# tayloraswift/swift-png

Hardware: NVIDIA H100
Metric: MPixels/s decode (inflate+unfilter) (higher is better)
Workload: dtype u8

## Files before the change

include/pngb200.h:

```cpp
#ifndef PNGB200_H
#define PNGB200_H

#include <stddef.h>
#include <stdint.h>

#ifdef __cplusplus
extern "C" {
#endif

#define PNGB200_VERSION 1

typedef enum pngb200_status {
    PNGB200_OK                                   = 0,
    PNGB200_NEED_MORE_INPUT                      = 1,
    PNGB200_ERR_STREAM_CHECKSUM                  = -1,
    PNGB200_ERR_BLOCK_TYPE                       = -2,
    PNGB200_ERR_BLOCK_COUNT_PARITY               = -3,
    PNGB200_ERR_RUNLITERAL_SYMBOL_COUNT          = -4,
    PNGB200_ERR_CODELENGTH_HUFFMAN_TABLE         = -5,
    PNGB200_ERR_CODELENGTH_SEQUENCE              = -6,
    PNGB200_ERR_HUFFMAN_TABLE                    = -7,
    PNGB200_ERR_STRING_REFERENCE                 = -8,
    PNGB200_ERR_INVALID_SYMBOL                   = -9,
    PNGB200_ERR_ZLIB_METHOD                      = -16,
// ... 46 lines not shown

typedef struct pngb200_ctx pngb200_ctx;

pngb200_ctx* pngb200_ctx_create(int device);
void         pngb200_ctx_destroy(pngb200_ctx* ctx);
int          pngb200_ctx_trim(pngb200_ctx* ctx);
const char*  pngb200_last_error(const pngb200_ctx* ctx);
void*        pngb200_ctx_stream(pngb200_ctx* ctx);
int          pngb200_ctx_device(const pngb200_ctx* ctx);
uint64_t     pngb200_ctx_launch_count(const pngb200_ctx* ctx);
void         pngb200_ctx_set_inflate_mode(pngb200_ctx* ctx, int mode);
int          pngb200_ctx_stage_ms(pngb200_ctx* ctx, float ms[3]);
int          pngb200_ctx_inflate_stats(pngb200_ctx* ctx, size_t count, uint64_t out[4]);
int          pngb200_ctx_inflate_counters(pngb200_ctx* ctx, size_t count, uint64_t out[24]);
int          pngb200_ctx_segment_stats(pngb200_ctx* ctx, uint64_t out[3]);
int          pngb200_ctx_last_inflate_engine(pngb200_ctx* ctx);
int          pngb200_ctx_filter_histogram(pngb200_ctx* ctx, uint64_t out[6]);


typedef struct pngb200_stream_desc {
    const uint8_t* src;
    size_t         src_len;
    uint8_t*       dst;
    size_t         dst_cap;
    int32_t        format;
    int32_t        status;
    uint32_t       err_a, err_b;
    uint32_t       checksum;
    uint32_t       blocks;
    uint64_t       produced;
// ... 164 lines not shown
```

swift-png_b200/__init__.py:

```python
from __future__ import annotations

import ctypes as C
import importlib.util
import os
from dataclasses import dataclass

from . import shard

_HERE = os.path.dirname(os.path.abspath(__file__))
LIB_PATH = os.environ.get("PNGB200_LIB") or os.path.join(_HERE, "libpngb200.so")
HEADER_PATH = os.path.join(_HERE, "..", "include", "pngb200.h")

OK = 0
NEED_MORE_INPUT = 1
ERR_STREAM_CHECKSUM = -1
ERR_BLOCK_TYPE = -2
ERR_BLOCK_COUNT_PARITY = -3
ERR_RUNLITERAL_SYMBOL_COUNT = -4
ERR_CODELENGTH_HUFFMAN_TABLE = -5
ERR_CODELENGTH_SEQUENCE = -6
ERR_HUFFMAN_TABLE = -7
ERR_STRING_REFERENCE = -8
ERR_INVALID_SYMBOL = -9
ERR_ZLIB_METHOD = -16
# ... 178 lines not shown
    L.pngb200_ctx_inflate_stats.argtypes = [C.c_void_p, C.c_size_t, C.POINTER(C.c_uint64)]
    L.pngb200_ctx_inflate_stats.restype = C.c_int
    L.pngb200_deflator_create.argtypes = [C.c_void_p, C.c_int, C.c_int, C.c_int, C.c_size_t]
    L.pngb200_deflator_create.restype = C.c_void_p
    L.pngb200_deflator_destroy.argtypes = [C.c_void_p]
    L.pngb200_deflator_destroy.restype = None
    L.pngb200_deflator_push.argtypes = [C.c_void_p, C.c_char_p, C.c_size_t, C.c_int]
    L.pngb200_deflator_push.restype = C.c_int
    for fn in (L.pngb200_deflator_pop, L.pngb200_deflator_pull):
        fn.argtypes = [C.c_void_p, C.POINTER(C.POINTER(C.c_uint8)), C.POINTER(C.c_size_t)]
        fn.restype = C.c_int
    L.pngb200_ctx_filter_histogram.argtypes = [C.c_void_p, C.POINTER(C.c_uint64)]
    L.pngb200_ctx_filter_histogram.restype = C.c_int
    L.pngb200_ctx_segment_stats.argtypes = [C.c_void_p, C.POINTER(C.c_uint64)]
    L.pngb200_ctx_segment_stats.restype = C.c_int
    if os.environ.get("PNGB200_LIB") is None or hasattr(L, "pngb200_ctx_last_inflate_engine"):
        L.pngb200_ctx_last_inflate_engine.argtypes = [C.c_void_p]
        L.pngb200_ctx_last_inflate_engine.restype = C.c_int
    L.pngb200_ctx_inflate_counters.argtypes = [C.c_void_p, C.c_size_t, C.POINTER(C.c_uint64)]
    L.pngb200_ctx_inflate_counters.restype = C.c_int
    L.pngb200_inflate_batch.argtypes = [C.c_void_p, C.POINTER(StreamDesc), C.c_size_t, C.c_int]
    L.pngb200_inflate_batch.restype = C.c_int
    for name in ("pngb200_decode_batch", "pngb200_decode_batch_enqueue", "pngb200_unfilter_batch"):
        getattr(L, name).argtypes = [C.c_void_p, C.POINTER(ImageDesc), C.c_size_t, C.c_int]
        getattr(L, name).restype = C.c_int
    L.pngb200_decode_batch_finish.argtypes = [C.c_void_p, C.POINTER(ImageDesc), C.c_size_t]
    L.pngb200_decode_batch_finish.restype = C.c_int
    L.pngb200_filter_batch.argtypes = [C.c_void_p, C.POINTER(FilterDesc), C.c_size_t, C.c_int]
    L.pngb200_filter_batch.restype = C.c_int
    L.pngb200_deflate_batch.argtypes = [C.c_void_p, C.POINTER(DeflateDesc), C.c_size_t, C.c_int]
# ... 86 lines not shown
                 "stored_blocks"]
        return dict(waves=out[0], walk_tokens=out[1], resolve_rounds=out[2], fallbacks=out[3], tokens=out[4],
                    matches=out[5], deferred_matches=out[6], blocks=out[7],
                    cycles={n: out[8 + i] for i, n in enumerate(names)})

    def filter_histogram(self):
        out = (C.c_uint64 * 6)()
        self.check(self._lib.pngb200_ctx_filter_histogram(self.handle, out))
        return list(out)

    def segment_stats(self):
        out = (C.c_uint64 * 3)()
        self.check(self._lib.pngb200_ctx_segment_stats(self.handle, out))
        return dict(streams=out[0], segments=out[1], fallbacks=out[2])

    def last_inflate_engine(self) -> str:
        if not hasattr(self._lib, "pngb200_ctx_last_inflate_engine"):
            return ""
        return {0: "inflate_parallel_kernel", 1: "inflate_wave_kernel", 2: "inflate_cells_kernel"}.get(
            self._lib.pngb200_ctx_last_inflate_engine(self.handle), "")

    def set_inflate_mode(self, mode: int):
        self._lib.pngb200_ctx_set_inflate_mode(self.handle, mode)

    def check(self, rc: int):
        if rc != OK:
            raise PNGB200Error(rc, self._lib.pngb200_last_error(self.handle).decode())


@dataclass
# ... 358 lines not shown
```

swift-png_b200/csrc/common.cuh:

```cuda
#pragma once

#ifdef PNGB200_EMU
#include "simt.h"
#else
#include <cuda_runtime.h>
#define PNGB200_DYN_SMEM(name) extern __shared__ __align__(16) unsigned char name[]
#endif
#include <stdint.h>

#include "../../include/pngb200.h"

namespace pngb200 {

struct StreamJob {
    const uint8_t* src;
    uint64_t       src_len;
    uint8_t*       dst;
    uint64_t       dst_cap;
    uint64_t       start_bit;
    uint64_t       start_out;
    int32_t        format;
    int32_t        phase;
    uint64_t       stop_bit;
    uint32_t       symbolic;
    uint32_t       pad_;
    uint8_t*       scratch;
    uint64_t       scratch_cap;
};

struct StreamResult {
    int32_t  status;
    uint32_t err_a, err_b;
    uint32_t checksum;
    uint32_t blocks;
    uint32_t declared;
    uint64_t produced;
    uint64_t consumed_bits;
    uint64_t resume_bit;
    uint64_t resume_out;
    uint32_t trailer_seen;
    uint32_t phase;
    uint32_t stat_waves, stat_sync_rounds, stat_resolve_rounds, stat_fallback;
    uint64_t stat_tokens, stat_matches, stat_deferred;
    uint32_t ck_done;
    uint32_t pad_;
    uint64_t stat_cycles[12];
};

struct ImageJob {
    const uint8_t*      filtered;
    uint8_t*            pixels;
    const StreamResult* inflated;
    uint64_t            filtered_len;
    uint32_t            width, height;
    uint32_t            pitch;
    uint8_t             volume, depth, interlaced, bpp;
};

__device__ __forceinline__ uint64_t usable_bytes(const StreamResult* r, uint64_t fallback)
{
    if (r == nullptr) return fallback;
// ... 26 lines not shown
```

swift-png_b200/csrc/inflate_segments.cuh:

```cuda
#pragma once

#include "common.cuh"
#include "inflate_wave.cuh"

namespace pngb200 {

constexpr uint32_t SEG_WINDOW = 32768;

struct SegmentRecord {
    const uint16_t* sym;
    uint8_t*        out;
    uint64_t        produced;
    uint32_t        stream;
    uint32_t        first;
};

__global__ void __launch_bounds__(256) window_propagate_kernel(const SegmentRecord* segs, const uint32_t* stream_first,
                                                               uint32_t nstreams, uint8_t* windows)
{
    if (blockIdx.x >= nstreams) return;
    const uint32_t lo = stream_first[blockIdx.x], hi = stream_first[blockIdx.x + 1];
    for (uint32_t k = lo; k + 1 < hi; ++k) {
        const SegmentRecord s  = segs[k];
        const uint8_t*      w  = windows + (size_t)k * SEG_WINDOW;
// ... 31 lines not shown
        const uint64_t i = base + j;
        if (i >= s.produced) break;
        const uint16_t x = s.sym[i];
        s.out[i] = (x & 0x8000u) ? (s.first ? 0 : w[x & 0x7fffu]) : (uint8_t)x;
    }
}

struct SplitRecord {
    const StreamResult* head;
    const StreamResult* tail;
    const uint16_t*     sym;
    uint8_t*            out;
    uint64_t            dst_cap;
    uint64_t            split_bit;
    StreamResult*       final_;
};

constexpr uint32_t SPLIT_CTAS = 64;

__device__ __forceinline__ bool split_lines_up(const SplitRecord& s, uint64_t n1, uint64_t n2)
{
    return s.head->status == PNGB200_OK && s.head->phase == 1 && s.head->consumed_bits == s.split_bit &&
           s.tail->status == PNGB200_OK && s.tail->phase == 2 && n1 >= SEG_WINDOW && n1 + n2 <= s.dst_cap;
}

__global__ void __launch_bounds__(256) split_resolve_kernel(const SplitRecord* recs, uint32_t* partial)
{
    const SplitRecord s  = recs[blockIdx.x];
    const uint64_t    n1 = s.head->produced, n2 = s.tail->produced;
    uint32_t*         pp = partial + 2 * ((size_t)blockIdx.x * SPLIT_CTAS + blockIdx.y);
    if (!split_lines_up(s, n1, n2)) return;
    const uint8_t* w = s.out + n1 - SEG_WINDOW;
    uint8_t*       o = s.out + n1;
    uint64_t a = 0, b = 0;
    for (uint64_t base = (uint64_t)blockIdx.y * 4096; base < n2; base += (uint64_t)SPLIT_CTAS * 4096) {
        for (uint32_t j = threadIdx.x; j < 4096; j += blockDim.x) {
            const uint64_t i = base + j;
            if (i >= n2) break;
            const uint16_t x = s.sym[i];
            const uint8_t  v = (x & 0x8000u) ? w[x & 0x7fffu] : (uint8_t)x;
            o[i] = v;
            a += v;
            b += (n2 - i) * v;
        }
        b %= ADLER_MOD32;
    }
    uint32_t a32 = (uint32_t)(a % ADLER_MOD32), b32 = (uint32_t)b;
    for (int k = 16; k; k >>= 1) {
        a32 += __shfl_down_sync(0xffffffffu, a32, k);
        b32 += __shfl_down_sync(0xffffffffu, b32, k);
    }
    __shared__ uint32_t red[2][8];
    const unsigned warp = threadIdx.x >> 5;
    if (lane_id() == 0) { red[0][warp] = a32 % ADLER_MOD32; red[1][warp] = b32 % ADLER_MOD32; }
    __syncthreads();
    if (threadIdx.x == 0) {
        uint32_t sa = 0, sb = 0;
        for (unsigned k = 0; k < blockDim.x / 32; ++k) { sa += red[0][k]; sb += red[1][k]; }
// ... 48 lines not shown
```

swift-png_b200/csrc/inflate_wave.cuh:

```cuda
#pragma once

#include "inflate_serial.cuh"

namespace pngb200 {

#ifndef WV_CTAS
#define WV_CTAS 2
#endif
constexpr int      WV_THREADS      = 256;
constexpr int      WV_CTAS_PER_SM  = WV_CTAS;
constexpr int      WV_WARPS        = WV_THREADS / 32;
constexpr uint32_t WV_SUB_BITS     = 256;
constexpr uint32_t WV_BITS         = WV_THREADS * WV_SUB_BITS;
constexpr uint32_t WV_WORDS        = WV_BITS / 32 + 8;
constexpr uint32_t WV_SMEM_WORDS   = WV_WORDS + WV_WORDS / 8 + 1;
constexpr uint32_t WV_RING         = 65536;
constexpr uint32_t WV_WINDOW       = 32768;
constexpr uint32_t WV_OUT_BYTES    = WV_RING - WV_WINDOW;
constexpr uint32_t WV_BITMAP_WORDS = WV_OUT_BYTES / 32;
constexpr uint32_t WV_LIST_CAP     = WV_BITS / 2 + 64;
constexpr uint64_t WV_MAX_WAVE_OUT = (uint64_t)WV_LIST_CAP * 258;
constexpr uint32_t WV_HDR_WORDS    = 192;
constexpr uint32_t ADLER_MOD32     = 65521;
#ifndef WV_POLL_NS
// ... 35 lines not shown
    uint32_t     wn_[WV_THREADS];
    uint64_t     cross_[WV_THREADS];
    uint16_t     wc_[WV_THREADS];
    uint16_t     next_[WV_THREADS];
    uint8_t      kind_[WV_THREADS];
    uint8_t      wlist[2][WV_THREADS];
    uint16_t     dpre_[WV_THREADS];
    uint16_t     cst_[WV_THREADS];
    uint32_t     dsum[WV_WARPS];
    uint32_t     wcount[3];
    uint32_t     bitmap[WV_BITMAP_WORDS];
    uint8_t      ring[WV_RING] __align__(16);
    uint64_t     warp_sums[WV_WARPS + 1];
    uint32_t     adler_a[WV_WARPS], adler_b[WV_WARPS];
    uint32_t     exc[WV_WARPS], valid[WV_WARPS];
    uint32_t     last, term, anomaly, ticket;
    uint64_t     cyc[12], tick;
    uint64_t     pf_bar;
    WvHeader     hdr;
};

struct WvParams {
    const StreamJob* jobs;
    StreamResult*    results;
    const uint32_t*  order;
    uint32_t*        ticket;
    uint8_t*         scratch;
    uint64_t         scratch_stride;
    uint64_t         bitmap_words;
    int              count;
};

struct CopyItem { uint32_t o; uint32_t run_dist; };

#ifdef PNGB200_EMU
typedef uintptr_t saddr_t;
inline uint32_t lds32(saddr_t addr) { return *(const uint32_t*)addr; }
inline uint32_t bfe32(uint32_t x, uint32_t pos, uint32_t len);
inline saddr_t smem_addr(const void* p) { return (uintptr_t)p; }
inline saddr_t opaque(saddr_t a) { return a; }
inline uint32_t bmsk(uint32_t pos, uint32_t width)
{
    pos &= 0xff; width &= 0xff;
    if (pos > 31 || width == 0) return 0;
    const uint32_t m = width >= 32 ? ~0u : (1u << width) - 1u;
// ... 482 lines not shown
        }
        __syncthreads();
        if (sh.ticket >= (uint32_t)P.count) return;
        const int       j   = P.order ? (int)P.order[sh.ticket] : (int)sh.ticket;
        const StreamJob job = P.jobs[j];
        StreamResult*   r   = P.results + j;

        BitReader br;
        br.init(job.src, job.src_len, job.start_bit);
        uint64_t out    = job.start_out;
        uint32_t blocks = 0, waves = 0, resolve_rounds = 0;
        uint64_t n_tokens = 0, n_matches = 0, n_deferred = 0, walk_tokens = 0;
        int      st     = PNGB200_OK;
        uint32_t phase  = (uint32_t)job.phase;
        uint64_t resume_bit = job.start_bit, resume_out = job.start_out;
        uint8_t* const dst = job.dst;
        const bool     sym = job.symbolic != 0;
        const uint32_t esz = sym ? 2u : 1u;
        const uint32_t mis = (uint32_t)((uintptr_t)dst & 15);
        bool fallback = false;
        bool ring_stale = job.start_out != 0;
        bool     pf_pending = false;
        uint64_t pf_first = 0;
        const bool adler_on = job.start_out == 0 && !sym;
        uint32_t   s1 = 1, s2 = 0;
        uint64_t   pend_len = 0;
        bool       pend = false;
        auto fold_adler = [&]() {
            if (pend && t == 0) {
                uint64_t A = 0, B = 0;
                for (int w = 0; w < WV_WARPS; ++w) { A += sh.adler_a[w]; B += sh.adler_b[w]; }
                s2 = (uint32_t)((s2 + (pend_len % ADLER_MOD32) * s1 + B) % ADLER_MOD32);
                s1 = (uint32_t)((s1 + A) % ADLER_MOD32);
            }
            pend = false;
// ... 6 lines not shown
            uint32_t a32 = (uint32_t)(a % ADLER_MOD32), b32 = (uint32_t)(bw % ADLER_MOD32);
            for (int o = 16; o; o >>= 1) {
                a32 += __shfl_down_sync(0xffffffffu, a32, o);
                b32 += __shfl_down_sync(0xffffffffu, b32, o);
            }
            if (lane == 0) { sh.adler_a[warp] = a32; sh.adler_b[warp] = b32; }
            pend = true;
            pend_len = n;
        };
        auto tick = [&](int i) {
            if (t == 0) {
                const uint64_t now = (uint64_t)clock64();
                sh.cyc[i] += now - sh.tick;
                sh.tick = now;
            }
        };

        if (phase == 0) {
            st = read_stream_header(br, job.format, r);
            if (st == PNGB200_OK) {
                resume_bit = br.at();
                phase = 1;
            }
        }
        if (st == PNGB200_OK && phase == 2) st = read_trailer(br, job.format, r);

        while (st == PNGB200_OK && phase == 1) {
            __syncthreads();
            fold_adler();
            {
// ... 18 lines not shown
            }
            __syncthreads();
            const WvHeader hdr = sh.hdr;
            st = hdr.status;
            if (st != PNGB200_OK) break;
            const int      type = hdr.type, final = hdr.final;
            const uint32_t stored = hdr.stored;
            br.seek(hdr.pos);
            if (type != 0) {
                st = build_block_tables(&sh.ser, r, hdr.nlit, hdr.ndist, (int)t, WV_THREADS);
                if (st != PNGB200_OK) break;
            }
            tick(0);
            if (type == 0) {
                if (!br.have(8 * (uint64_t)stored)) { st = PNGB200_NEED_MORE_INPUT; break; }
                if (out + stored > job.dst_cap) { st = fail(r, PNGB200_ERR_OUTPUT_CAPACITY); break; }
                const uint8_t* s = job.src + (br.at() >> 3);
                if (sym) for (uint32_t k = t; k < stored; k += WV_THREADS) reinterpret_cast<uint16_t*>(dst)[out + k] = s[k];
                else for (uint32_t k = t; k < stored; k += WV_THREADS) dst[out + k] = s[k];
                if (adler_on && stored) adler_hbm(s, stored);
                if (stored) ring_stale = true;
                out += stored;
                br.seek(br.pos + 8 * (uint64_t)stored);
                __syncthreads();
                fold_adler();
                tick(9);
            } else {
                bool block_done = false;
                while (!block_done) {
                    ++waves;
                    const uint64_t wstart = br.pos;
                    const uint64_t wbase  = (wstart >> 5) & ~(uint64_t)7;
                    __syncthreads();
                    bool staged = false;
                    if (pf_pending) {
                        while (!mbar_try_wait(&sh.pf_bar, pf_parity)) {}
                        pf_parity ^= 1;
                        pf_pending = false;
                        if (wbase >= pf_first && wbase - pf_first < 4) {
                            const uint32_t* lin = sh.mask + (uint32_t)(wbase - pf_first);
// ... 221 lines not shown
                        uint64_t ws = lane < WV_WARPS ? sh.warp_sums[lane] : 0, wi = ws;
                        for (int o = 1; o < 32; o <<= 1) {
                            uint64_t v = __shfl_up_sync(0xffffffffu, wi, o);
                            if ((int)lane >= o) wi += v;
                        }
                        if (lane < WV_WARPS) sh.warp_sums[lane] = wi - ws;
                        if (lane == WV_WARPS - 1) sh.warp_sums[WV_WARPS] = wi;
                    }
                    __syncthreads();
                    tick(5);
                    const uint64_t excl    = sh.warp_sums[warp] + incl - mine;
                    const uint32_t o_start = (uint32_t)(excl & 0xffffffffffull);
                    const uint32_t c_start = (uint32_t)(excl >> 40);
                    const uint64_t total64 = sh.warp_sums[WV_WARPS] & 0xffffffffffull;
                    const uint32_t np      = (uint32_t)(sh.warp_sums[WV_WARPS] >> 40);
                    if (sh.anomaly || out + total64 > job.dst_cap || total64 > P.bitmap_words * 32) {
                        fallback = true;
                        break;
                    }
                    const uint32_t  total  = (uint32_t)total64;
                    {
                        const uint64_t nbase = wbase + WV_BITS / 32;
                        const uint64_t first = nbase - ((((uintptr_t)br.words >> 2) + nbase) & 3);
                        if (first >= 1 && (first + WV_PF_WORDS + 1) * 32 <= br.total_bits) {
                            if (t == 0) {
                                fence_proxy_async();
                                mbar_expect_tx(&sh.pf_bar, sizeof(uint32_t) * WV_PF_WORDS);
                                bulk_g2s(sh.mask, br.words + first, sizeof(uint32_t) * WV_PF_WORDS, &sh.pf_bar);
                            }
                            pf_pending = true;
                            pf_first = first;
                        }
// ... 107 lines not shown
                            ++rounds;
                            if (!__any_sync(0xffffffffu, g < nd)) break;
                            if (!__any_sync(0xffffffffu, progressed)) __nanosleep(WV_POLL_NS);
                        }
                        resolve_rounds += rounds;
                        WV_COUNT(4, rounds);
                    }
                    __threadfence_block();
                    __syncthreads();
                    tick(7);
                    if (sh.anomaly) {
                        for (uint32_t k = t; k < (total + 31) / 32; k += WV_THREADS) U[k] = 0;
                        fallback = true;
                        break;
                    }
                    if (!in_hbm && total) {
                        const uint32_t shift = rbase & 15u;
                        uint8_t* const gbase = wdst - shift;
                        const uint32_t rb16  = rbase - shift;
                        const uint32_t end   = shift + total;
                        const uint32_t nq    = (end + 15) >> 4;
                        uint32_t a = 0, bw = 0;
                        for (uint32_t c = t; c < nq; c += WV_THREADS) {
                            const uint32_t lo = c << 4, hi = lo + 16;
                            if (lo >= shift && hi <= end) {
                                const uint4 x = *reinterpret_cast<const uint4*>(sh.ring + ((rb16 + lo) & 0xffffu));
                                reinterpret_cast<uint4*>(gbase)[c] = x;
                                adler_chunk16_u32(x, end - lo, a, bw);
                            } else {
                                for (uint32_t k = max(lo, shift); k < min(hi, end); ++k) {
// ... 12 lines not shown
                            }
                            if (lane == 0) { sh.adler_a[warp] = a32; sh.adler_b[warp] = b32; }
                            pend = true;
                            pend_len = total;
                        }
                    } else if (in_hbm && adler_on) {
                        adler_hbm(wdst, total);
                    }
                    tick(8);
                    out += total;
                    if (t == 0) n_matches += np;
                    n_tokens += emitted;
                    n_deferred += deferred;
                    br.seek((wbase << 5) + sh.wpos_[last]);
                    if (term == WK_EOB || term == WK_OWN_EOB) block_done = true;
                }
                if (fallback) break;
            }
            ++blocks;
            resume_bit = br.at();
            resume_out = out;
            if (job.stop_bit && !final && br.at() >= job.stop_bit) break;
            if (final) {
                phase = 2;
                st = read_trailer(br, job.format, r);
                break;
            }
        }
        if (pf_pending) {
            while (!mbar_try_wait(&sh.pf_bar, pf_parity)) {}
// ... 25 lines not shown
                for (int w = 0; w < WV_WARPS; ++w) {
                    tk += sh.warp_sums[w];
                    df += sh.adler_a[w];
                    wt += sh.adler_b[w];
                    rr = max(rr, sh.exc[w]);
                }
                r->stat_waves          = waves;
                r->stat_sync_rounds    = (uint32_t)min(wt, (uint64_t)0xffffffffu);
                r->stat_resolve_rounds = rr;
                r->stat_tokens         = tk;
                r->stat_matches        = n_matches;
                r->stat_deferred       = df;
                for (int k = 0; k < 12; ++k) r->stat_cycles[k] = sh.cyc[k];
            }
        }
        if (fallback && sym) {
            if (t == 0) {
                r->status = PNGB200_ERR_INTERNAL;
                r->produced = out;
                r->consumed_bits = br.at();
                r->blocks = blocks;
            }
        } else if (fallback) {
            __syncthreads();
            if (warp == 0) serial_inflate(sh.ser, job, r, resume_bit, resume_out, 1, blocks);
        } else if (t == 0) {
            if (r->status == 0) r->status = st;
            r->produced      = out;
            r->consumed_bits = br.at();
            r->blocks        = blocks;
            r->resume_bit    = resume_bit;
            r->resume_out    = resume_out;
            r->phase         = phase;
            if (adler_on && job.format != PNGB200_FORMAT_GZIP) {
                const uint32_t computed = s2 << 16 | s1;
                r->checksum = computed;
                r->ck_done  = 1;
                if (r->trailer_seen && job.format != PNGB200_FORMAT_IOS && r->status >= 0 && r->declared != computed) {
                    r->status = PNGB200_ERR_STREAM_CHECKSUM;
                    r->err_a  = r->declared;
                    r->err_b  = computed;
                }
            }
        }
        if (t == 0) r->stat_fallback = fallback ? 1u : 0u;
    }
}

#ifndef PNGB200_EMU
inline int configure_inflate_wave()
{
    return (int)cudaFuncSetAttribute(inflate_wave_kernel, cudaFuncAttributeMaxDynamicSharedMemorySize,
                                     (int)sizeof(WvShared));
}
#endif

inline uint64_t wv_bitmap_words(uint64_t max_dst_cap)
{
    uint64_t bytes = max_dst_cap < WV_MAX_WAVE_OUT ? max_dst_cap : WV_MAX_WAVE_OUT;
    return (bytes + 31) / 32 + 8;
// ... 9 lines not shown
```

swift-png_b200/csrc/pngb200_api.cu:

```cuda
#include <cuda_runtime.h>

#include <algorithm>
#include <cstdarg>
#include <cstdio>
#include <cstdlib>
#include <cstring>
#include <functional>
#include <string>
#include <thread>
#include <vector>

#include "checksum.cuh"
#include "common.cuh"
#include "deflate.cuh"
#include "filter.cuh"
#include "color.cuh"
#include "crc32.cuh"
#include "inflate_wave.cuh"
#include "inflate_parallel.cuh"
#include "inflate_cells.cuh"
#include "block_search.cuh"
#include "inflate_segments.cuh"
#include "inflate_serial.cuh"
#include "unfilter.cuh"
// ... 66 lines not shown
    cudaStream_t stream = nullptr;
    uint64_t     launches = 0;
    int          inflate_mode = 0;
    int          last_engine = -1;
    bool         cells_auto = false;
    bool         cells_segments = true;
    int          sm_count = 132;
    size_t       device_bytes = 0;
    std::string  error;
    bool         pending = false;
    int          pending_memspace = 0;
    DevBuf d_jobs, d_results, d_imgjobs, d_genjobs, d_misc, d_partial, d_filtered, d_in, d_out, d_order, d_scratch, d_dfscratch, d_dfjobs, d_dfres, d_enc,
           d_file, d_crc, d_seg, d_crctab, d_sgjobs, d_sgres, d_sgsym, d_sgsearch, d_sgrec, d_sgwin;
    PinBuf h_jobs, h_results, h_imgjobs, h_genjobs, h_misc, h_order, h_crc, h_seg, h_sgsearch, h_sgjobs, h_sgres, h_sgrec;
    uint64_t seg_streams = 0, seg_segments = 0, seg_fallbacks = 0;
    uint64_t scratch_stride = 0;
    size_t parallel_threshold = 8192;
    unsigned long long* d_hist = nullptr;
    size_t peer_streams = 0;
    bool   split = true;
    size_t plan_slots = 0;
    cudaEvent_t ev[4] = {nullptr, nullptr, nullptr, nullptr};
    std::vector<uint64_t> expected;
    std::vector<size_t>   out_offset;
    std::vector<size_t>   out_bytes;
    std::vector<pngb200_ctx*> lanes;
    std::function<int()> bulk_h2d;
};

namespace {
// ... 219 lines not shown
        StreamResult* hf = ctx->h_sgres.as<StreamResult>();
        for (size_t a = 0; a < accepted.size(); ++a) {
            hf[a] = finals[a];
            CU(cudaMemcpyAsync(d_results + accepted[a], hf + a, sizeof(StreamResult), cudaMemcpyHostToDevice, ctx->stream));
        }
        std::vector<uint32_t> rest;
        for (uint32_t i : par)
            if (std::find(accepted.begin(), accepted.end(), i) == accepted.end()) rest.push_back(i);
        par.swap(rest);
    }
    return PNGB200_OK;
}

size_t plan_slots(const pngb200_ctx* ctx) { return ctx->plan_slots ? ctx->plan_slots : (size_t)ctx->sm_count * WV_CTAS_PER_SM; }

constexpr double kSymbolicCost = 1.38;


double split_head_share(const pngb200_ctx* ctx, const StreamJob* h_jobs, const std::vector<uint32_t>& par)
{
    constexpr uint64_t kMinSplit = 1u << 20;
    const size_t slots = plan_slots(ctx), nb = par.size();
    if (!ctx->split || ctx->peer_streams || nb * 2 <= slots || nb >= slots) return 0;
    const double h = nb * kSymbolicCost / ((double)(slots - nb) + nb * kSymbolicCost);
    if (h < 0.55 || h > 0.95) return 0;
    for (uint32_t i : par) {
        const StreamJob& j = h_jobs[i];
        if (j.format != PNGB200_FORMAT_ZLIB || j.start_bit != 0 || j.phase != 0 || j.src_len < kMinSplit || j.dst_cap < kMinSplit ||
            !j.scratch || (uintptr_t)j.scratch % 16 || (double)j.scratch_cap < 2.5 * (1.0 - h) * (double)j.dst_cap + 4096)
            return 0;
    }
// ... 9 lines not shown
    for (size_t k = 0; k < nb; ++k) {
        const StreamJob& j = h_jobs[par[k]];
        sj[k] = SearchJob{j.src, j.src_len, (uint64_t)(h * (double)(8 * j.src_len)), 8 * j.src_len, ~0ull};
    }
    CU(cudaMemcpyAsync(ctx->d_sgsearch.p, sj, sizeof(SearchJob) * nb, cudaMemcpyHostToDevice, ctx->stream));
    block_search_kernel<<<dim3((unsigned)nb, BS_CTAS), 256, 0, ctx->stream>>>(ctx->d_sgsearch.as<SearchJob>(), (uint32_t)nb);
    ctx->launches++;
    CU(cudaMemcpyAsync(sj, ctx->d_sgsearch.p, sizeof(SearchJob) * nb, cudaMemcpyDeviceToHost, ctx->stream));
    CU(cudaStreamSynchronize(ctx->stream));
    std::vector<uint32_t> cut, rest;
    for (size_t k = 0; k < nb; ++k) (sj[k].found != ~0ull ? cut : rest).push_back(par[k]);
    const size_t n = cut.size();
    if (n == 0) return PNGB200_OK;
    CU(ctx->h_sgjobs.reserve(sizeof(StreamJob) * 2 * n));
    CU(ctx->d_sgjobs.reserve(sizeof(StreamJob) * 2 * n));
    CU(ctx->d_sgres.reserve(sizeof(StreamResult) * 2 * n));
    StreamJob* sg = ctx->h_sgjobs.as<StreamJob>();
    uint64_t max_cap = 0;
    for (size_t k = 0, s = 0; k < nb; ++k) {
        if (sj[k].found == ~0ull) continue;
        const StreamJob& j = h_jobs[par[k]];
        StreamJob& hd = sg[s];
        StreamJob& tl = sg[n + s];
        ++s;
        hd = j;
        hd.stop_bit = sj[k].found;
        tl = j;
        tl.start_bit = sj[k].found;
        tl.phase = 1;
        tl.symbolic = 1;
        tl.dst = j.scratch;
        tl.dst_cap = j.scratch_cap / 2 - 64;
        max_cap = std::max(max_cap, j.dst_cap);
    }
    CU(cudaMemcpyAsync(ctx->d_sgjobs.p, sg, sizeof(StreamJob) * 2 * n, cudaMemcpyHostToDevice, ctx->stream));
    CU(cudaMemsetAsync(ctx->d_sgres.p, 0, sizeof(StreamResult) * 2 * n, ctx->stream));
    {
        WvParams pp;
        pp.bitmap_words = wv_bitmap_words(max_cap);
        pp.scratch_stride = wv_scratch_stride(pp.bitmap_words);
        const unsigned grid = (unsigned)std::min<size_t>(2 * n, slots);
        const size_t need = (size_t)pp.scratch_stride * grid + 256;
        if (need > ctx->d_scratch.cap || pp.scratch_stride != ctx->scratch_stride) {
            CU(ctx->d_scratch.reserve(need));
            CU(cudaMemsetAsync(ctx->d_scratch.p, 0, ctx->d_scratch.cap, ctx->stream));
            ctx->scratch_stride = pp.scratch_stride;
        }
        pp.ticket = (uint32_t*)((char*)ctx->d_scratch.p + (size_t)pp.scratch_stride * grid);
        CU(cudaMemsetAsync(pp.ticket, 0, sizeof(uint32_t), ctx->stream));
        pp.jobs = ctx->d_sgjobs.as<StreamJob>();
        pp.results = ctx->d_sgres.as<StreamResult>();
        pp.order = nullptr;
        pp.scratch = ctx->d_scratch.as<uint8_t>();
        pp.count = (int)(2 * n);
        inflate_wave_kernel<<<grid, WV_THREADS, sizeof(WvShared), ctx->stream>>>(pp);
        ctx->launches++;
    }
    const size_t off_accept  = align_up(sizeof(SplitRecord) * n, 256);
    const size_t off_partial = align_up(off_accept + sizeof(uint32_t) * n, 256);
    const size_t table       = off_partial + sizeof(uint32_t) * 2 * SPLIT_CTAS * n;
    CU(ctx->h_sgrec.reserve(off_partial));
    CU(ctx->d_sgrec.reserve(table));
    SplitRecord* rec = ctx->h_sgrec.as<SplitRecord>();
    const StreamResult* d_sgres = ctx->d_sgres.as<StreamResult>();
    for (size_t s = 0; s < n; ++s) {
        const StreamJob& j = h_jobs[cut[s]];
        rec[s] = SplitRecord{d_sgres + s, d_sgres + n + s, (const uint16_t*)j.scratch, j.dst, j.dst_cap, sg[s].stop_bit,
                             ctx->d_results.as<StreamResult>() + cut[s]};
    }
    CU(cudaMemcpyAsync(ctx->d_sgrec.p, rec, sizeof(SplitRecord) * n, cudaMemcpyHostToDevice, ctx->stream));
    const SplitRecord* d_rec = ctx->d_sgrec.as<SplitRecord>();
    uint32_t* d_accept  = (uint32_t*)((char*)ctx->d_sgrec.p + off_accept);
    uint32_t* d_partial = (uint32_t*)((char*)ctx->d_sgrec.p + off_partial);
    split_resolve_kernel<<<dim3((unsigned)n, SPLIT_CTAS), 256, 0, ctx->stream>>>(d_rec, d_partial);
    split_finish_kernel<<<(unsigned)((n + 127) / 128), 128, 0, ctx->stream>>>(d_rec, (uint32_t)n, d_partial, d_accept);
    ctx->launches += 2;
    CU(cudaGetLastError());
    uint32_t* accept = (uint32_t*)((char*)ctx->h_sgrec.p + off_accept);
    CU(cudaMemcpyAsync(accept, d_accept, sizeof(uint32_t) * n, cudaMemcpyDeviceToHost, ctx->stream));
    CU(cudaStreamSynchronize(ctx->stream));
    ctx->seg_streams += n;
    ctx->seg_segments += 2 * n;
    for (size_t s = 0; s < n; ++s)
        if (!accept[s]) {
            ctx->seg_fallbacks++;
            rest.push_back(cut[s]);
        }
    std::vector<uint32_t> left;
    for (uint32_t i : par)
        if (std::find(rest.begin(), rest.end(), i) != rest.end()) left.push_back(i);
    par.swap(left);
    return PNGB200_OK;
}

int run_inflate(pngb200_ctx* ctx, const StreamJob* h_jobs, size_t count)
{
    ctx->last_engine = -1;
    StreamJob*    d_jobs    = ctx->d_jobs.as<StreamJob>();
    StreamResult* d_results = ctx->d_results.as<StreamResult>();
    ctx->seg_streams = ctx->seg_segments = ctx->seg_fallbacks = 0;
    CU(cudaMemsetAsync(d_results, 0, sizeof(StreamResult) * count, ctx->stream));
    auto before_first_launch = [&]() -> int {
        int rc = PNGB200_OK;
        if (ctx->bulk_h2d) {
            rc = ctx->bulk_h2d();
            ctx->bulk_h2d = nullptr;
        }
        if (rc == PNGB200_OK) CU(cudaEventRecord(ctx->ev[0], ctx->stream));
        return rc;
    };
    {
        std::vector<uint32_t> par, ser;
        for (size_t i = 0; i < count; ++i) {
            bool big = h_jobs[i].src_len >= ctx->parallel_threshold;
            if (ctx->inflate_mode == 1) big = false;
// ... 530 lines not shown
    DeviceGuard guard(ctx->device);
    std::vector<pngb200_ctx*> all{ctx};
    all.insert(all.end(), ctx->lanes.begin(), ctx->lanes.end());
    for (pngb200_ctx* c : all) {
        if (!c->d_hist) continue;
        unsigned long long h[6];
        CU(cudaStreamSynchronize(c->stream));
        CU(cudaMemcpy(h, c->d_hist, sizeof h, cudaMemcpyDeviceToHost));
        for (int k = 0; k < 6; ++k) out[k] += h[k];
    }
    return PNGB200_OK;
}

int pngb200_ctx_last_inflate_engine(pngb200_ctx* ctx) { return ctx ? ctx->last_engine : -1; }

int pngb200_ctx_segment_stats(pngb200_ctx* ctx, uint64_t out[3])
{
    if (!ctx || !out) return PNGB200_ERR_BAD_ARGUMENT;
    out[0] = ctx->seg_streams;
    out[1] = ctx->seg_segments;
    out[2] = ctx->seg_fallbacks;
    return PNGB200_OK;
}

int pngb200_ctx_stage_ms(pngb200_ctx* ctx, float ms[3])
{
    if (!ctx || !ms) return PNGB200_ERR_BAD_ARGUMENT;
    DeviceGuard guard(ctx->device);
    for (int i = 0; i < 3; ++i)
        if (cudaEventElapsedTime(&ms[i], ctx->ev[i], ctx->ev[i + 1]) != cudaSuccess) {
// ... 32 lines not shown
                CU(cudaMemcpyAsync(ctx->d_in.as<uint8_t>() + in_off[i], s[i].src, s[i].src_len,
                                   cudaMemcpyHostToDevice, ctx->stream));
    }
    for (size_t i = 0; i < count; ++i) {
        bool host = memspace == PNGB200_MEM_HOST;
        jobs[i].src = host ? ctx->d_in.as<uint8_t>() + in_off[i] : s[i].src;
        jobs[i].src_len = s[i].src_len;
        jobs[i].dst = host ? ctx->d_out.as<uint8_t>() + out_off[i] : s[i].dst;
        jobs[i].dst_cap = s[i].dst_cap;
        jobs[i].start_bit = 0;
        jobs[i].start_out = 0;
        jobs[i].format = s[i].format;
        jobs[i].phase = 0;
        jobs[i].stop_bit = 0;
        jobs[i].symbolic = 0;
        jobs[i].pad_ = 0;
        jobs[i].scratch = nullptr;
        jobs[i].scratch_cap = 0;
    }
    CU(cudaMemcpyAsync(ctx->d_jobs.p, jobs, sizeof(StreamJob) * count, cudaMemcpyHostToDevice, ctx->stream));
    int rc = run_inflate(ctx, jobs, count);
    if (rc != PNGB200_OK) return rc;
    CU(cudaMemcpyAsync(ctx->h_results.p, ctx->d_results.p, sizeof(StreamResult) * count,
                       cudaMemcpyDeviceToHost, ctx->stream));
    CU(cudaStreamSynchronize(ctx->stream));
    const StreamResult* r = ctx->h_results.as<StreamResult>();
    for (size_t i = 0; i < count; ++i) {
        s[i].status = r[i].status;
        s[i].err_a = r[i].err_a;
        s[i].err_b = r[i].err_b;
        s[i].checksum = r[i].checksum;
// ... 53 lines not shown
            return PNGB200_OK;
        };
    }
    StreamJob* jobs = ctx->h_jobs.as<StreamJob>();
    for (size_t i = 0; i < count; ++i) {
        jobs[i].src = host ? ctx->d_in.as<uint8_t>() + in_off[i] : im[i].idat;
        jobs[i].src_len = im[i].idat_len;
        jobs[i].dst = ctx->d_filtered.as<uint8_t>() + f_off[i];
        jobs[i].dst_cap = geo[i].filtered + 16;
        jobs[i].start_bit = 0;
        jobs[i].start_out = 0;
        jobs[i].format = im[i].format;
        jobs[i].phase = 0;
        jobs[i].stop_bit = 0;
        jobs[i].symbolic = 0;
        jobs[i].pad_ = 0;
        jobs[i].scratch = host ? nullptr : im[i].pixels;
        jobs[i].scratch_cap = host ? 0 : im[i].pixels_cap;
    }
    CU(cudaMemcpyAsync(ctx->d_jobs.p, jobs, sizeof(StreamJob) * count, cudaMemcpyHostToDevice, ctx->stream));
    int rc = run_inflate(ctx, jobs, count);
    ctx->bulk_h2d = nullptr;
    if (rc != PNGB200_OK) return rc;
    std::vector<UnfilterItem> items(count);
    for (size_t i = 0; i < count; ++i) {
        UnfilterItem& it = items[i];
        it.filtered = jobs[i].dst;
        it.filtered_mut = jobs[i].dst;
        it.pixels = host ? ctx->d_out.as<uint8_t>() + ctx->out_offset[i] : im[i].pixels;
        it.inflated = ctx->d_results.as<StreamResult>() + i;
        it.filtered_len = 0;
// ... 599 lines not shown
    CU(z->h_res.reserve(sizeof(StreamResult) + sizeof(StreamJob)));
    int rc = inflator_grow_out(z, std::max<size_t>(1 << 16, z->produced + 4 * n + 1024));
    if (rc != PNGB200_OK) return rc;
    for (;;) {
        StreamJob* job = (StreamJob*)((char*)z->h_res.p + sizeof(StreamResult));
        job->src = z->d_in.as<uint8_t>();
        job->src_len = z->input.size();
        job->dst = z->d_out.as<uint8_t>();
        job->dst_cap = z->d_out.cap;
        job->start_bit = z->resume_bit;
        job->start_out = z->resume_out;
        job->format = z->format;
        job->phase = (int32_t)z->phase;
        job->stop_bit = 0;
        job->symbolic = 0;
        job->pad_ = 0;
        CU(cudaMemcpyAsync(z->d_job.p, job, sizeof(StreamJob), cudaMemcpyHostToDevice, ctx->stream));
        CU(cudaMemsetAsync(z->d_res.p, 0, sizeof(StreamResult), ctx->stream));
        const uint64_t pending = z->input.size() - std::min<uint64_t>(z->input.size(), z->resume_bit >> 3);
        if (pending >= (64u << 10)) {
            const uint64_t bitmap_words = wv_bitmap_words(job->dst_cap);
            const uint64_t stride = wv_scratch_stride(bitmap_words);
            const size_t   need = (size_t)stride + 256;
            if (need > ctx->d_scratch.cap || stride != ctx->scratch_stride) {
                CU(ctx->d_scratch.reserve(need));
                CU(cudaMemsetAsync(ctx->d_scratch.p, 0, ctx->d_scratch.cap, ctx->stream));
                ctx->scratch_stride = stride;
            }
            uint32_t* ticket = (uint32_t*)((char*)ctx->d_scratch.p + (size_t)stride);
            CU(cudaMemsetAsync(ticket, 0, sizeof(uint32_t), ctx->stream));
            WvParams pp;
// ... 95 lines not shown
```

Measured before the change: 9955.

## Let speculative tail inflate switch from symbolic to plain bytes once window resolved

The tail segment of a split stream is decoded symbolically (16-bit entries referencing the unknown head window). Once no unresolved back-references remain within the last window, the wave kernel now converts the last window to bytes and continues emitting plain 8-bit output into a fresh region of the scratch buffer, recording the switch point. The split resolve kernel then resolves only the symbolic prefix and copies the byte suffix with vectorized funnel-shift loads while folding Adler-32. This halves output traffic for the late part of the tail, at the cost of an extra per-wave max-mark reduction and a barrier. The symbolic cost constant used to size the head/tail split is lowered to match, and split statistics plus a host copy of the piece results are added.

```diff
diff --git a/include/pngb200.h b/include/pngb200.h
--- a/include/pngb200.h
+++ b/include/pngb200.h
@@ -84,6 +84,7 @@
 int          pngb200_ctx_inflate_stats(pngb200_ctx* ctx, size_t count, uint64_t out[4]);
 int          pngb200_ctx_inflate_counters(pngb200_ctx* ctx, size_t count, uint64_t out[24]);
 int          pngb200_ctx_segment_stats(pngb200_ctx* ctx, uint64_t out[3]);
+int          pngb200_ctx_split_stats(pngb200_ctx* ctx, uint64_t out[6]);
 int          pngb200_ctx_last_inflate_engine(pngb200_ctx* ctx);
 int          pngb200_ctx_filter_histogram(pngb200_ctx* ctx, uint64_t out[6]);
 
diff --git a/swift-png_b200/__init__.py b/swift-png_b200/__init__.py
--- a/swift-png_b200/__init__.py
+++ b/swift-png_b200/__init__.py
@@ -216,6 +216,9 @@
     L.pngb200_ctx_filter_histogram.restype = C.c_int
     L.pngb200_ctx_segment_stats.argtypes = [C.c_void_p, C.POINTER(C.c_uint64)]
     L.pngb200_ctx_segment_stats.restype = C.c_int
+    if os.environ.get("PNGB200_LIB") is None or hasattr(L, "pngb200_ctx_split_stats"):
+        L.pngb200_ctx_split_stats.argtypes = [C.c_void_p, C.POINTER(C.c_uint64)]
+        L.pngb200_ctx_split_stats.restype = C.c_int
     if os.environ.get("PNGB200_LIB") is None or hasattr(L, "pngb200_ctx_last_inflate_engine"):
         L.pngb200_ctx_last_inflate_engine.argtypes = [C.c_void_p]
         L.pngb200_ctx_last_inflate_engine.restype = C.c_int
@@ -332,6 +335,12 @@
         self.check(self._lib.pngb200_ctx_segment_stats(self.handle, out))
         return dict(streams=out[0], segments=out[1], fallbacks=out[2])
 
+    def split_stats(self):
+        out = (C.c_uint64 * 6)()
+        self.check(self._lib.pngb200_ctx_split_stats(self.handle, out))
+        return dict(head_bytes=out[0], head_cycles=out[1], tail_bytes=out[2], tail_cycles=out[3], switched=out[4],
+                    symbolic_bytes=out[5])
+
     def last_inflate_engine(self) -> str:
         if not hasattr(self._lib, "pngb200_ctx_last_inflate_engine"):
             return ""
diff --git a/swift-png_b200/csrc/common.cuh b/swift-png_b200/csrc/common.cuh
--- a/swift-png_b200/csrc/common.cuh
+++ b/swift-png_b200/csrc/common.cuh
@@ -23,7 +23,7 @@
     int32_t        phase;
     uint64_t       stop_bit;
     uint32_t       symbolic;
-    uint32_t       pad_;
+    uint32_t       may_switch;
     uint8_t*       scratch;
     uint64_t       scratch_cap;
 };
@@ -45,6 +45,11 @@
     uint32_t ck_done;
     uint32_t pad_;
     uint64_t stat_cycles[12];
+};
+
+struct SwitchRecord {
+    uint64_t out;
+    uint64_t bytes;
 };
 
 struct ImageJob {
diff --git a/swift-png_b200/csrc/inflate_segments.cuh b/swift-png_b200/csrc/inflate_segments.cuh
--- a/swift-png_b200/csrc/inflate_segments.cuh
+++ b/swift-png_b200/csrc/inflate_segments.cuh
@@ -69,14 +69,18 @@
     uint64_t            dst_cap;
     uint64_t            split_bit;
     StreamResult*       final_;
+    const SwitchRecord* sw = nullptr;
 };
+
+__device__ __forceinline__ uint64_t split_switch_out(const SplitRecord& s, uint64_t n2) { return s.sw ? s.sw->out : n2; }
 
 constexpr uint32_t SPLIT_CTAS = 64;
 
 __device__ __forceinline__ bool split_lines_up(const SplitRecord& s, uint64_t n1, uint64_t n2)
 {
     return s.head->status == PNGB200_OK && s.head->phase == 1 && s.head->consumed_bits == s.split_bit &&
-           s.tail->status == PNGB200_OK && s.tail->phase == 2 && n1 >= SEG_WINDOW && n1 + n2 <= s.dst_cap;
+           s.tail->status == PNGB200_OK && s.tail->phase == 2 && n1 >= SEG_WINDOW && n1 + n2 <= s.dst_cap &&
+           split_switch_out(s, n2) <= n2;
 }
 
 __global__ void __launch_bounds__(256) split_resolve_kernel(const SplitRecord* recs, uint32_t* partial)
@@ -85,18 +89,47 @@
     const uint64_t    n1 = s.head->produced, n2 = s.tail->produced;
     uint32_t*         pp = partial + 2 * ((size_t)blockIdx.x * SPLIT_CTAS + blockIdx.y);
     if (!split_lines_up(s, n1, n2)) return;
+    const uint64_t m = split_switch_out(s, n2);
     const uint8_t* w = s.out + n1 - SEG_WINDOW;
     uint8_t*       o = s.out + n1;
+    const uint8_t* bytes = reinterpret_cast<const uint8_t*>(s.sym) + (s.sw ? s.sw->bytes : 0);
     uint64_t a = 0, b = 0;
     for (uint64_t base = (uint64_t)blockIdx.y * 4096; base < n2; base += (uint64_t)SPLIT_CTAS * 4096) {
-        for (uint32_t j = threadIdx.x; j < 4096; j += blockDim.x) {
-            const uint64_t i = base + j;
-            if (i >= n2) break;
+        const uint64_t end = min(base + 4096, n2);
+        for (uint64_t i = base + threadIdx.x; i < min(end, m); i += blockDim.x) {
             const uint16_t x = s.sym[i];
             const uint8_t  v = (x & 0x8000u) ? w[x & 0x7fffu] : (uint8_t)x;
             o[i] = v;
             a += v;
             b += (n2 - i) * v;
+        }
+        if (end > m) {
+            const uint64_t  lo = max(base, m);
+            const uintptr_t g0 = (uintptr_t)(o + lo) & ~(uintptr_t)15;
+            const uint64_t  ng = ((uintptr_t)(o + end) - g0 + 15) / 16;
+            for (uint64_t g = threadIdx.x; g < ng; g += blockDim.x) {
+                const int64_t i0 = (int64_t)(g0 + 16 * g - (uintptr_t)o);
+                if (i0 >= (int64_t)lo && (uint64_t)i0 + 16 <= end) {
+                    const uint8_t*  src = bytes + ((uint64_t)i0 - m);
+                    const uint32_t* sw  = reinterpret_cast<const uint32_t*>((uintptr_t)src & ~(uintptr_t)3);
+                    const uint32_t  sh  = 8 * (uint32_t)((uintptr_t)src & 3);
+                    const uint32_t  w0 = sw[0], w1 = sw[1], w2 = sw[2], w3 = sw[3], w4 = sw[4];
+                    uint4 x;
+                    x.x = __funnelshift_r(w0, w1, sh);
+                    x.y = __funnelshift_r(w1, w2, sh);
+                    x.z = __funnelshift_r(w2, w3, sh);
+                    x.w = __funnelshift_r(w3, w4, sh);
+                    *reinterpret_cast<uint4*>(o + i0) = x;
+                    adler_chunk16(x, n2 - (uint64_t)i0, a, b);
+                } else {
+                    for (int64_t i = max(i0, (int64_t)lo); i < min(i0 + 16, (int64_t)end); ++i) {
+                        const uint8_t v = bytes[i - m];
+                        o[i] = v;
+                        a += v;
+                        b += (n2 - i) * v;
+                    }
+                }
+            }
         }
         b %= ADLER_MOD32;
     }
diff --git a/swift-png_b200/csrc/inflate_wave.cuh b/swift-png_b200/csrc/inflate_wave.cuh
--- a/swift-png_b200/csrc/inflate_wave.cuh
+++ b/swift-png_b200/csrc/inflate_wave.cuh
@@ -73,6 +73,7 @@
     uint64_t     warp_sums[WV_WARPS + 1];
     uint32_t     adler_a[WV_WARPS], adler_b[WV_WARPS];
     uint32_t     exc[WV_WARPS], valid[WV_WARPS];
+    uint32_t     mark[WV_WARPS];
     uint32_t     last, term, anomaly, ticket;
     uint64_t     cyc[12], tick;
     uint64_t     pf_bar;
@@ -88,6 +89,7 @@
     uint64_t         scratch_stride;
     uint64_t         bitmap_words;
     int              count;
+    SwitchRecord*    switched = nullptr;
 };
 
 struct CopyItem { uint32_t o; uint32_t run_dist; };
@@ -600,11 +602,14 @@
         int      st     = PNGB200_OK;
         uint32_t phase  = (uint32_t)job.phase;
         uint64_t resume_bit = job.start_bit, resume_out = job.start_out;
-        uint8_t* const dst = job.dst;
-        const bool     sym = job.symbolic != 0;
-        const uint32_t esz = sym ? 2u : 1u;
-        const uint32_t mis = (uint32_t)((uintptr_t)dst & 15);
-        bool fallback = false;
+        uint8_t* dst     = job.dst;
+        uint64_t dst_cap = job.dst_cap;
+        bool     sym     = job.symbolic != 0;
+        uint32_t esz     = sym ? 2u : 1u;
+        uint32_t mis     = (uint32_t)((uintptr_t)dst & 15);
+        const bool may_switch = sym && job.may_switch;
+        uint64_t   mark_end = 0, sw_out = ~0ull, sw_bytes = 0;
+        bool fallback = false, over_cap = false;
         bool ring_stale = job.start_out != 0;
         bool     pf_pending = false;
         uint64_t pf_first = 0;
@@ -641,6 +646,24 @@
                 sh.cyc[i] += now - sh.tick;
                 sh.tick = now;
             }
+        };
+        auto try_switch = [&]() {
+            if (!may_switch || !sym || out < mark_end + WV_WINDOW) return;
+            const uint64_t area = (2 * out + 15) & ~(uint64_t)15;
+            const uint64_t room = 2 * job.dst_cap;
+            if (area + WV_WINDOW > room) return;
+            const uint16_t* const s16 = reinterpret_cast<const uint16_t*>(job.dst);
+            uint8_t* const        nd  = job.dst + area + WV_WINDOW - out;
+            for (uint64_t x = out - WV_WINDOW + t; x < out; x += WV_THREADS) nd[x] = (uint8_t)s16[x];
+            __syncthreads();
+            sym        = false;
+            esz        = 1;
+            dst        = nd;
+            dst_cap    = room - area - WV_WINDOW + out;
+            mis        = (uint32_t)((uintptr_t)nd & 15);
+            ring_stale = true;
+            sw_out     = out;
+            sw_bytes   = area + WV_WINDOW;
         };
 
         if (phase == 0) {
@@ -689,7 +712,7 @@
             tick(0);
             if (type == 0) {
                 if (!br.have(8 * (uint64_t)stored)) { st = PNGB200_NEED_MORE_INPUT; break; }
-                if (out + stored > job.dst_cap) { st = fail(r, PNGB200_ERR_OUTPUT_CAPACITY); break; }
+                if (out + stored > dst_cap) { st = fail(r, PNGB200_ERR_OUTPUT_CAPACITY); break; }
                 const uint8_t* s = job.src + (br.at() >> 3);
                 if (sym) for (uint32_t k = t; k < stored; k += WV_THREADS) reinterpret_cast<uint16_t*>(dst)[out + k] = s[k];
                 else for (uint32_t k = t; k < stored; k += WV_THREADS) dst[out + k] = s[k];
@@ -699,6 +722,7 @@
                 br.seek(br.pos + 8 * (uint64_t)stored);
                 __syncthreads();
                 fold_adler();
+                try_switch();
                 tick(9);
             } else {
                 bool block_done = false;
@@ -950,8 +974,9 @@
                     const uint32_t c_start = (uint32_t)(excl >> 40);
                     const uint64_t total64 = sh.warp_sums[WV_WARPS] & 0xffffffffffull;
                     const uint32_t np      = (uint32_t)(sh.warp_sums[WV_WARPS] >> 40);
-                    if (sh.anomaly || out + total64 > job.dst_cap || total64 > P.bitmap_words * 32) {
+                    if (sh.anomaly || out + total64 > dst_cap || total64 > P.bitmap_words * 32) {
                         fallback = true;
+                        over_cap = out + total64 > dst_cap;
                         break;
                     }
                     const uint32_t  total  = (uint32_t)total64;
@@ -1089,6 +1114,19 @@
                         fallback = true;
                         break;
                     }
+                    if (may_switch && sym) {
+                        const uint16_t* const ws = reinterpret_cast<const uint16_t*>(wdst);
+                        uint32_t lm = 0;
+                        for (uint32_t k = t; k < total; k += WV_THREADS)
+                            if (ws[k] & 0x8000u) lm = k + 1;
+                        for (int o = 16; o; o >>= 1) lm = max(lm, __shfl_xor_sync(0xffffffffu, lm, o));
+                        if (lane == 0) sh.mark[warp] = lm;
+                        __syncthreads();
+                        uint32_t wm = 0;
+#pragma unroll
+                        for (int w = 0; w < WV_WARPS; ++w) wm = max(wm, sh.mark[w]);
+                        if (wm) mark_end = out + wm;
+                    }
                     if (!in_hbm && total) {
                         const uint32_t shift = rbase & 15u;
                         uint8_t* const gbase = wdst - shift;
@@ -1131,6 +1169,7 @@
                     n_deferred += deferred;
                     br.seek((wbase << 5) + sh.wpos_[last]);
                     if (term == WK_EOB || term == WK_OWN_EOB) block_done = true;
+                    try_switch();
                 }
                 if (fallback) break;
             }
@@ -1186,9 +1225,9 @@
                 for (int k = 0; k < 12; ++k) r->stat_cycles[k] = sh.cyc[k];
             }
         }
-        if (fallback && sym) {
+        if (fallback && job.symbolic) {
             if (t == 0) {
-                r->status = PNGB200_ERR_INTERNAL;
+                r->status = sw_out != ~0ull && over_cap ? PNGB200_ERR_OUTPUT_CAPACITY : PNGB200_ERR_INTERNAL;
                 r->produced = out;
                 r->consumed_bits = br.at();
                 r->blocks = blocks;
@@ -1216,6 +1255,7 @@
             }
         }
         if (t == 0) r->stat_fallback = fallback ? 1u : 0u;
+        if (t == 0 && may_switch && P.switched) P.switched[j] = SwitchRecord{sw_out != ~0ull ? sw_out : out, sw_bytes};
     }
 }
 
diff --git a/swift-png_b200/csrc/pngb200_api.cu b/swift-png_b200/csrc/pngb200_api.cu
--- a/swift-png_b200/csrc/pngb200_api.cu
+++ b/swift-png_b200/csrc/pngb200_api.cu
@@ -104,6 +104,7 @@
            d_file, d_crc, d_seg, d_crctab, d_sgjobs, d_sgres, d_sgsym, d_sgsearch, d_sgrec, d_sgwin;
     PinBuf h_jobs, h_results, h_imgjobs, h_genjobs, h_misc, h_order, h_crc, h_seg, h_sgsearch, h_sgjobs, h_sgres, h_sgrec;
     uint64_t seg_streams = 0, seg_segments = 0, seg_fallbacks = 0;
+    uint64_t split_stats[6] = {};
     uint64_t scratch_stride = 0;
     size_t parallel_threshold = 8192;
     unsigned long long* d_hist = nullptr;
@@ -353,7 +354,7 @@
 
 size_t plan_slots(const pngb200_ctx* ctx) { return ctx->plan_slots ? ctx->plan_slots : (size_t)ctx->sm_count * WV_CTAS_PER_SM; }
 
-constexpr double kSymbolicCost = 1.38;
+constexpr double kSymbolicCost = 1.05;
 
 
 double split_head_share(const pngb200_ctx* ctx, const StreamJob* h_jobs, const std::vector<uint32_t>& par)
@@ -393,7 +394,9 @@
     if (n == 0) return PNGB200_OK;
     CU(ctx->h_sgjobs.reserve(sizeof(StreamJob) * 2 * n));
     CU(ctx->d_sgjobs.reserve(sizeof(StreamJob) * 2 * n));
-    CU(ctx->d_sgres.reserve(sizeof(StreamResult) * 2 * n));
+    const size_t res_bytes = sizeof(StreamResult) * 2 * n + sizeof(SwitchRecord) * 2 * n;
+    static_assert(sizeof(StreamResult) % alignof(SwitchRecord) == 0, "switch records behind the results");
+    CU(ctx->d_sgres.reserve(res_bytes));
     StreamJob* sg = ctx->h_sgjobs.as<StreamJob>();
     uint64_t max_cap = 0;
     for (size_t k = 0, s = 0; k < nb; ++k) {
@@ -408,12 +411,14 @@
         tl.start_bit = sj[k].found;
         tl.phase = 1;
         tl.symbolic = 1;
+        tl.may_switch = 1;
         tl.dst = j.scratch;
         tl.dst_cap = j.scratch_cap / 2 - 64;
         max_cap = std::max(max_cap, j.dst_cap);
     }
     CU(cudaMemcpyAsync(ctx->d_sgjobs.p, sg, sizeof(StreamJob) * 2 * n, cudaMemcpyHostToDevice, ctx->stream));
-    CU(cudaMemsetAsync(ctx->d_sgres.p, 0, sizeof(StreamResult) * 2 * n, ctx->stream));
+    CU(cudaMemsetAsync(ctx->d_sgres.p, 0, res_bytes, ctx->stream));
+    SwitchRecord* d_switch = (SwitchRecord*)(ctx->d_sgres.as<StreamResult>() + 2 * n);
     {
         WvParams pp;
         pp.bitmap_words = wv_bitmap_words(max_cap);
@@ -432,6 +437,7 @@
         pp.order = nullptr;
         pp.scratch = ctx->d_scratch.as<uint8_t>();
         pp.count = (int)(2 * n);
+        pp.switched = d_switch;
         inflate_wave_kernel<<<grid, WV_THREADS, sizeof(WvShared), ctx->stream>>>(pp);
         ctx->launches++;
     }
@@ -445,7 +451,7 @@
     for (size_t s = 0; s < n; ++s) {
         const StreamJob& j = h_jobs[cut[s]];
         rec[s] = SplitRecord{d_sgres + s, d_sgres + n + s, (const uint16_t*)j.scratch, j.dst, j.dst_cap, sg[s].stop_bit,
-                             ctx->d_results.as<StreamResult>() + cut[s]};
+                             ctx->d_results.as<StreamResult>() + cut[s], d_switch + n + s};
     }
     CU(cudaMemcpyAsync(ctx->d_sgrec.p, rec, sizeof(SplitRecord) * n, cudaMemcpyHostToDevice, ctx->stream));
     const SplitRecord* d_rec = ctx->d_sgrec.as<SplitRecord>();
@@ -457,14 +463,30 @@
     CU(cudaGetLastError());
     uint32_t* accept = (uint32_t*)((char*)ctx->h_sgrec.p + off_accept);
     CU(cudaMemcpyAsync(accept, d_accept, sizeof(uint32_t) * n, cudaMemcpyDeviceToHost, ctx->stream));
+    CU(ctx->h_sgres.reserve(res_bytes));
+    CU(cudaMemcpyAsync(ctx->h_sgres.p, d_sgres, res_bytes, cudaMemcpyDeviceToHost, ctx->stream));
     CU(cudaStreamSynchronize(ctx->stream));
     ctx->seg_streams += n;
     ctx->seg_segments += 2 * n;
-    for (size_t s = 0; s < n; ++s)
+    const StreamResult* pieces = ctx->h_sgres.as<StreamResult>();
+    const SwitchRecord* switched = (const SwitchRecord*)(pieces + 2 * n);
+    for (size_t s = 0; s < n; ++s) {
         if (!accept[s]) {
             ctx->seg_fallbacks++;
             rest.push_back(cut[s]);
-        }
+            continue;
+        }
+        const StreamResult &hd = pieces[s], &tl = pieces[n + s];
+        ctx->split_stats[0] += hd.produced;
+        ctx->split_stats[2] += tl.produced;
+        for (int q = 0; q < 12; ++q) {
+            ctx->split_stats[1] += hd.stat_cycles[q];
+            ctx->split_stats[3] += tl.stat_cycles[q];
+        }
+        const SwitchRecord& sw = switched[n + s];
+        ctx->split_stats[4] += sw.out < tl.produced;
+        ctx->split_stats[5] += sw.out;
+    }
     std::vector<uint32_t> left;
     for (uint32_t i : par)
         if (std::find(rest.begin(), rest.end(), i) != rest.end()) left.push_back(i);
@@ -478,6 +500,7 @@
     StreamJob*    d_jobs    = ctx->d_jobs.as<StreamJob>();
     StreamResult* d_results = ctx->d_results.as<StreamResult>();
     ctx->seg_streams = ctx->seg_segments = ctx->seg_fallbacks = 0;
+    for (uint64_t& v : ctx->split_stats) v = 0;
     CU(cudaMemsetAsync(d_results, 0, sizeof(StreamResult) * count, ctx->stream));
     auto before_first_launch = [&]() -> int {
         int rc = PNGB200_OK;
@@ -1038,6 +1061,13 @@
 
 int pngb200_ctx_last_inflate_engine(pngb200_ctx* ctx) { return ctx ? ctx->last_engine : -1; }
 
+int pngb200_ctx_split_stats(pngb200_ctx* ctx, uint64_t out[6])
+{
+    if (!ctx || !out) return PNGB200_ERR_BAD_ARGUMENT;
+    for (int k = 0; k < 6; ++k) out[k] = ctx->split_stats[k];
+    return PNGB200_OK;
+}
+
 int pngb200_ctx_segment_stats(pngb200_ctx* ctx, uint64_t out[3])
 {
     if (!ctx || !out) return PNGB200_ERR_BAD_ARGUMENT;
@@ -1100,7 +1130,7 @@
         jobs[i].phase = 0;
         jobs[i].stop_bit = 0;
         jobs[i].symbolic = 0;
-        jobs[i].pad_ = 0;
+        jobs[i].may_switch = 0;
         jobs[i].scratch = nullptr;
         jobs[i].scratch_cap = 0;
     }
@@ -1184,7 +1214,7 @@
         jobs[i].phase = 0;
         jobs[i].stop_bit = 0;
         jobs[i].symbolic = 0;
-        jobs[i].pad_ = 0;
+        jobs[i].may_switch = 0;
         jobs[i].scratch = host ? nullptr : im[i].pixels;
         jobs[i].scratch_cap = host ? 0 : im[i].pixels_cap;
     }
@@ -1814,7 +1844,7 @@
         job->phase = (int32_t)z->phase;
         job->stop_bit = 0;
         job->symbolic = 0;
-        job->pad_ = 0;
+        job->may_switch = 0;
         CU(cudaMemcpyAsync(z->d_job.p, job, sizeof(StreamJob), cudaMemcpyHostToDevice, ctx->stream));
         CU(cudaMemsetAsync(z->d_res.p, 0, sizeof(StreamResult), ctx->stream));
         const uint64_t pending = z->input.size() - std::min<uint64_t>(z->input.size(), z->resume_bit >> 3);
```

Result: faster. 10480, median of 6 (+5.3%).
